# taleinat/fuzzysearch

Hardware: NVIDIA H100
Metric: haystack_GB_per_s_scanned (higher is better)
Workload: dtype u8

## Files before the change

fuzzysearch_b200/csrc/api.cu:

```cuda
#include <algorithm>
#include <atomic>
#include <cstdarg>
#include <cstdio>
#include <cmath>
#include <cstring>
#include <dlfcn.h>
#include <sched.h>
#include <unistd.h>
#include <condition_variable>
#include <memory>
#include <mutex>
#include <thread>
#include <new>
#include <string>
#include <type_traits>
#include <vector>

#include "kernels.cuh"
#include "ham_kernels.cuh"
#include "lp_kernels.cuh"
#include "post_kernels.cuh"
#include "p2p_kernels.cuh"
#include "batch_kernels.cuh"
#include "ham_batch_kernels.cuh"
// ... 8 lines not shown

static thread_local std::string g_err;

static int fail(int code, const char *fmt, ...) {
    char buf[512];
    va_list ap;
    va_start(ap, fmt);
    vsnprintf(buf, sizeof buf, fmt, ap);
    va_end(ap);
    g_err = buf;
    return code;
}

#define CK(call)                                                                          \
    do {                                                                                  \
        cudaError_t e_ = (call);                                                          \
        if (e_ != cudaSuccess)                                                            \
            return fail(FZB_E_CUDA, "%s failed: %s", #call, cudaGetErrorString(e_));      \
    } while (0)

#define TRY(call)                                                                         \
    do {                                                                                  \
        const int rc_ = (call);                                                           \
        if (rc_) return rc_;                                                              \
    } while (0)

enum class Mem { Device, Pinned, Mapped };

template <class T, Mem kMem>
class Buf {
  public:
    Buf() = default;
    Buf(Buf &&o) noexcept : p_(o.p_), n_(o.n_) {
        o.p_ = nullptr;
        o.n_ = 0;
    }
    Buf &operator=(Buf o) noexcept {
        std::swap(p_, o.p_);
        std::swap(n_, o.n_);
        return *this;
    }
    ~Buf() {
        if (p_) (void)(kMem == Mem::Device ? cudaFree(p_) : cudaFreeHost(p_));
    }
    T *get() const { return p_; }
    uint64_t size() const { return n_; }
    explicit operator bool() const { return p_ != nullptr; }
    T &operator[](uint64_t i) const {
        static_assert(kMem != Mem::Device, "device memory is not addressable from the host");
        return p_[i];
    }
    int alloc(uint64_t n, uint64_t bytes = 0) {
        Buf b;
        if (!bytes) bytes = n * sizeof(T);
        const unsigned flags = kMem == Mem::Mapped ? cudaHostAllocMapped | cudaHostAllocPortable : cudaHostAllocDefault;
        const cudaError_t e = kMem == Mem::Device ? cudaMalloc(&b.p_, bytes) : cudaHostAlloc(&b.p_, bytes, flags);
        if (e != cudaSuccess)
            return fail(FZB_E_CUDA, "%s(%llu bytes) failed: %s", kMem == Mem::Device ? "cudaMalloc" : "cudaHostAlloc",
                        (unsigned long long)bytes, cudaGetErrorString(e));
        b.n_ = n;
        *this = std::move(b);
        return FZB_OK;
    }

  private:
    T *p_ = nullptr;
    uint64_t n_ = 0;
};
template <class T> using DevBuf = Buf<T, Mem::Device>;
template <class T> using PinnedBuf = Buf<T, Mem::Pinned>;
template <class T> using MappedBuf = Buf<T, Mem::Mapped>;

struct BatchBufs {
    DevBuf<uint32_t> d_mbits;
    DevBuf<uint2> d_gtab;
    DevBuf<uint32_t> d_postings, d_pinfo;
    DevBuf<BatchPat> d_bpats;
    DevBuf<unsigned long long> d_mset;
    DevBuf<WorkItem> d_mwork;
};
struct LpBatchBufs {
    DevBuf<ulonglong2> d_lmlut;
    DevBuf<unsigned long long> d_lmlist;
    DevBuf<unsigned long long> d_lmkept;
    DevBuf<uint32_t> d_lmhist;
};
struct GenericBatchBufs {
    DevBuf<uint32_t> d_glim;
};
struct PeerBufs {
    DevBuf<uint8_t> d_p2p;
    DevBuf<MergeScratch> d_ms;
    DevBuf<unsigned long long> d_mscore;
    DevBuf<uint32_t> d_mpos;
    MappedBuf<int64_t> h_grows;
    MappedBuf<uint32_t> h_ghdr;
};
struct RecBufs {
    DevBuf<uint64_t> d_off;
    DevBuf<uint32_t> d_first;
    uint64_t longest = 0;
};
struct BestBufs {
    DevBuf<uint64_t> d_words;
    DevBuf<uint32_t> d_ids;
};
struct BestState {
    uint64_t *best, *top2;
    const uint32_t *ordinal;
};
struct NearBufs {
    DevBuf<uint64_t> d_head;
    DevBuf<uint64_t> d_words;
};
struct NearBatchBufs {
    DevBuf<uint32_t> d_lanes;
    DevBuf<uint8_t> d_pats;
    DevBuf<uint64_t> d_words;
    DevBuf<uint64_t> d_aux;
};
struct GatherBufs {
    uint32_t cap = 0;
    DevBuf<int64_t> d_send, d_recv;
    PinnedBuf<int64_t> h_send, h_recv;
};

template <class G, class F>
static int ensure_group(std::unique_ptr<G> &slot, F init) {
    if (slot) return FZB_OK;
    std::unique_ptr<G> g(new (std::nothrow) G());
    if (!g) return fail(FZB_E_CUDA, "out of host memory");
    TRY(init(*g));
    slot = std::move(g);
    return FZB_OK;
}

extern "C" int fzb_version(void) { return FZB_VERSION; }

extern "C" int fzb_device_count(void) {
    int n = 0;
    if (cudaGetDeviceCount(&n) != cudaSuccess) {
        cudaGetLastError();
        return 0;
    }
    return n;
}

extern "C" const char *fzb_last_error(void) { return g_err.c_str(); }

struct NcclId {
    char b[FZB_NCCL_ID_BYTES];
};
struct NcclApi {
    int (*GetUniqueId)(NcclId *id) = nullptr;
    int (*CommInitRank)(void **comm, int nranks, NcclId id, int rank) = nullptr;
    int (*AllGather)(const void *send, void *recv, size_t count, int dtype, void *comm, cudaStream_t s) = nullptr;
    int (*CommDestroy)(void *comm) = nullptr;
    const char *(*GetErrorString)(int) = nullptr;
    bool ok = false;
};
static NcclApi g_nccl;
static std::string g_nccl_path;

extern "C" void fzb_nccl_set_library(const char *path) { g_nccl_path = path ? path : ""; }

static int nccl_load() {
    static std::once_flag once;
// ... 1822 lines not shown
        if (rc > 0)
            for (uint32_t id : ids) drop(id);
        return rc < 0 ? rc : FZB_OK;
    }

    int finish_pass(const std::vector<RawRec> &raw, uint32_t n, const std::vector<uint32_t> &ids, fzb_stats pass,
                    int raw_order, bool unconsolidated) {
        if (!best) return split_batch(raw, ids, pass, raw_order, unconsolidated, out, &sum);
        if (n) {
            std::vector<uint32_t> ordinals(ids.size());
            for (size_t j = 0; j < ids.size(); j++) ordinals[j] = best->ordinal[ids[j]];
            CK(cudaMemcpyAsync(h->bestb->d_ids.get(), ordinals.data(), ordinals.size() * sizeof(uint32_t),
                               cudaMemcpyHostToDevice, h->stream));
            TRY(best_accumulate(h, *best, n, h->bestb->d_ids.get(), 0));
            pass.n_launches++;
        }
        for (uint32_t id : ids) done[id] = 1;
        add_stats(&sum, pass);
        return FZB_OK;
    }

    int finish(fzb_stats *total) {
        const uint32_t f = (flags & ~FZB_F_PER_RECORD) | (best ? FZB_F_NO_FINAL : 0u);
        for (uint32_t i = 0; i < count; i++) {
            if (settled(i)) continue;
            fzb_result *res = nullptr;
            auto planned = [&](Plan &pl) { pl = plans[i]; return FZB_OK; };
            TRY(settle(run_search(h, patterns + offsets[i], f, &res, planned), {}));
            if (!best) {
                add_stats(&sum, res->stats);
                out[i] = res;
                continue;
            }
            const int rc = best_accumulate(h, *best, res->raw_n, nullptr, best->ordinal[i]);
            if (res->raw_n) res->stats.n_launches++;
            add_stats(&sum, res->stats);
            fzb_result_destroy(res);
            TRY(rc);
        }
        sum.route = 7;
        if (total) *total = sum;
        return FZB_OK;
    }
};

template <class F>
static int run_batch_pass(const BatchCall &c, F enqueue, std::vector<RawRec> &raw, uint32_t cnts[CNT_COUNT],
                          fzb_stats &pass) {
    fzb_haystack *h = c.h;
    detach_pending(h);
    for (int attempt = 0; attempt < 8; attempt++) {
        h->counters_clean = false;
        CK(cudaMemsetAsync(h->d_counters.get(), 0, CNT_COUNT * sizeof(uint32_t), h->stream));
        CK(cudaEventRecord(h->ev[0], h->stream));
        int rc = enqueue();
        if (rc) return rc;
        CK(cudaEventRecord(h->ev[2], h->stream));
        rc = read_counters(h, cnts);
        if (rc) return rc;
        if (cnts[CNT_OVERFLOW]) return 1;
        const uint32_t n = cnts[CNT_OUT];
        if (n > kMaxRawRecs) return 1;
        if (n > h->d_out.size()) {
            TRY(ensure_out_cap(h, n));
            continue;
        }
        if (!c.best) raw.resize(n);
        if (!raw.empty()) {
            CK(cudaMemcpyAsync(raw.data(), h->d_out.get(), (size_t)n * sizeof(RawRec), cudaMemcpyDeviceToHost, h->stream));
            CK(cudaStreamSynchronize(h->stream));
        }
        float ms = 0.f;
        cudaEventElapsedTime(&ms, h->ev[0], h->ev[2]);
        pass.gpu_ms = ms;
        pass.bytes_scanned = h->buf_len;
        return FZB_OK;
    }
    return fail(FZB_E_CUDA, "output buffer kept overflowing");
}

struct ChunkSums {
    float scan_ms = 0.f;
    uint64_t listed = 0;
    uint32_t chunks = 0;
};

template <class S, class V>
static int run_chunks(fzb_haystack *h, uint64_t chunk, int list, int full, uint32_t cnts[CNT_COUNT], ChunkSums &s,
                      S scan, V verify) {
    s = ChunkSums{};
    for (uint64_t lo = h->own_lo; lo < h->own_hi; lo += chunk) {
        CK(cudaMemsetAsync(h->d_counters.get() + list, 0, 2 * sizeof(uint32_t), h->stream));
        CK(cudaEventRecord(h->ev[1], h->stream));
        scan(lo, std::min<uint64_t>(h->own_hi, lo + chunk));
        CK(cudaEventRecord(h->ev[2], h->stream));
        TRY(verify());
        CK(cudaGetLastError());
        s.chunks++;
        TRY(read_counters(h, cnts));
        float ms = 0.f;
        cudaEventElapsedTime(&ms, h->ev[1], h->ev[2]);
        s.scan_ms += ms;
        s.listed += cnts[list];
        if (cnts[CNT_OVERFLOW] || cnts[full]) return 1;
    }
    return FZB_OK;
}

static void fill_pat(BatchPat &bp, const BatchCall &c, uint32_t id) {
    memset(&bp, 0, sizeof bp);
    memcpy(bp.P, c.patterns + c.offsets[id], c.len(id));
    bp.m = (int)c.len(id);
    bp.k = (int)c.plans[id].k;
}

template <class F>
static int upload_pass_tables(fzb_haystack *h, const std::unordered_map<uint32_t, std::vector<uint32_t>> &grams,
                              const std::vector<uint32_t> &bits, const std::vector<uint32_t> &pinfo,
                              const std::vector<BatchPat> &pats, F mark) {
    std::vector<uint32_t> postings;
    std::vector<uint2> gtab(kGtabSlots, make_uint2(0, 0));
    for (auto &g : grams) {
        const uint32_t w = g.first;
        mark(w);
        for (size_t first = 0; first < g.second.size(); first += 255) {
            const uint32_t c = (uint32_t)std::min<size_t>(255, g.second.size() - first);
            uint32_t slot = (w * kGramMul) & (kGtabSlots - 1);
            while (gtab[slot].y != 0u) slot = (slot + 1) & (kGtabSlots - 1);
            gtab[slot] = make_uint2(w, (uint32_t)postings.size() | (c << 24));
            postings.insert(postings.end(), g.second.begin() + first, g.second.begin() + first + c);
        }
    }
    TRY(ensure_batch_buffers(h));
    BatchBufs &b = *h->batch;
    CK(cudaMemcpyAsync(b.d_mbits.get(), bits.data(), bits.size() * 4, cudaMemcpyHostToDevice, h->stream));
    CK(cudaMemcpyAsync(b.d_gtab.get(), gtab.data(), gtab.size() * sizeof(uint2), cudaMemcpyHostToDevice, h->stream));
    CK(cudaMemcpyAsync(b.d_postings.get(), postings.data(), postings.size() * 4, cudaMemcpyHostToDevice, h->stream));
    CK(cudaMemcpyAsync(b.d_pinfo.get(), pinfo.data(), pinfo.size() * 4, cudaMemcpyHostToDevice, h->stream));
    CK(cudaMemcpyAsync(b.d_bpats.get(), pats.data(), pats.size() * sizeof(BatchPat), cudaMemcpyHostToDevice, h->stream));
    return FZB_OK;
}

static MultiParams pass_params(const fzb_haystack *h) {
    MultiParams mp{};
    mp.H = h->d;
    mp.buf_lo = (int64_t)h->buf_lo;
    mp.buf_len = (int64_t)h->buf_len;
    mp.N = (int64_t)h->global_len;
    mp.own_lo = (int64_t)h->own_lo;
    mp.own_hi = (int64_t)h->own_hi;
    mp.bits = h->batch->d_mbits.get();
    mp.gtab = h->batch->d_gtab.get();
    mp.gtab_mask = kGtabSlots - 1;
    mp.postings = h->batch->d_postings.get();
    mp.pinfo = h->batch->d_pinfo.get();
    mp.counters = h->d_counters.get();
    return mp;
}

constexpr int kGenericBatchCap = 256;

static int prepare_generic_pass(const BatchCall &c, const std::vector<uint32_t> &ids, int grid) {
    fzb_haystack *h = c.h;
    TRY(ensure_group(h->gbatch, [](GenericBatchBufs &g) -> int { return g.d_glim.alloc(kMaxBatchPats); }));
    std::vector<uint32_t> lim;
    for (uint32_t id : ids) lim.push_back(c.plans[id].subs | c.plans[id].ins << 8 | c.plans[id].dels << 16);
    CK(cudaMemcpyAsync(h->gbatch->d_glim.get(), lim.data(), lim.size() * 4, cudaMemcpyHostToDevice, h->stream));
    return ensure_scratch(h, (uint64_t)grid * kLpThreads * 2 * kGenericBatchCap);
}

static int ensure_mhits(fzb_haystack *h) {
    if (h->d_mhits) return FZB_OK;
    DevBuf<unsigned long long> hits;
    TRY(hits.alloc(1u << 23));
    CK(cudaFuncSetAttribute(k_filter_mdense, cudaFuncAttributeMaxDynamicSharedMemorySize, (int)kMdenseSmem));
    h->d_mhits = std::move(hits);
    return FZB_OK;
}

static void two_bit_code(const uint8_t *patterns, const uint32_t *offsets, const std::vector<uint32_t> &ids,
                         uint8_t code[256]) {
    uint64_t freq[256] = {0};
    for (uint32_t id : ids)
        for (uint32_t b = offsets[id]; b < offsets[id + 1]; b++) freq[patterns[b]]++;
    int order[256];
    for (int c = 0; c < 256; c++) order[c] = c;
// ... 64 lines not shown
    const int64_t nvec = (int64_t)(round_up(h->buf_len, 16) / 16);
    const int64_t ntiles = (nvec + kMultiTileVecs - 1) / kMultiTileVecs;
    std::vector<RawRec> raw;
    uint32_t cnts[CNT_COUNT];
    fzb_stats pass{};
    const RecSet rs = rec_set(h);
    rc = run_batch_pass(c, [&]() -> int {
        MdenseParams dp{mp, b.d_bpats.get(), h->d_mhits.get(), hits_cap};
        if (ntiles > 0) {
            const int grid = (int)std::min<int64_t>(ntiles, h->sm_count);
            if (dense)
                k_filter_mdense<<<grid, kMultiThreads, kMdenseSmem, h->stream>>>(dp, nvec, ntiles);
            else
                k_filter_multi<<<grid, kMultiThreads, kMultiSmem, h->stream>>>(mp, nvec, ntiles);
        }
        CK(cudaEventRecord(h->ev[1], h->stream));
        with_recs(h, [&](auto rec) {
            constexpr bool R = decltype(rec)::value;
            if (generic && dense)
                k_verify_mhits_generic<R><<<ggrid, kLpThreads, 0, h->stream>>>(
                    dp, h->gbatch->d_glim.get(), h->d_scratch.get(), kGenericBatchCap, h->d_out.get(), h->d_out.size(),
                    h->d_counters.get(), rs);
            else if (generic)
                k_verify_multi_generic<R><<<ggrid, kLpThreads, 0, h->stream>>>(
                    mp, b.d_bpats.get(), h->gbatch->d_glim.get(), h->d_scratch.get(), kGenericBatchCap, h->d_out.get(),
                    h->d_out.size(), h->d_counters.get(), rs);
            else if (dense)
                k_verify_mhits<R><<<h->sm_count * 8, kMhThreads, 0, h->stream>>>(dp, h->d_out.get(), h->d_out.size(),
                                                                                    h->d_counters.get(), rs);
            else
                k_verify_multi<R><<<h->sm_count * 8, kVmThreads, 0, h->stream>>>(
                    mp, b.d_bpats.get(), h->d_out.get(), h->d_out.size(), h->d_counters.get(), rs);
        });
        CK(cudaGetLastError());
        return FZB_OK;
    }, raw, cnts, pass);
    if (rc > 0 && !dense) {
        CK(cudaMemsetAsync(b.d_mset.get(), 0, b.d_mset.size() * sizeof(unsigned long long), h->stream));
        CK(cudaStreamSynchronize(h->stream));
    }
    if (rc) return rc;
    float filter_ms = 0.f;
    cudaEventElapsedTime(&filter_ms, h->ev[0], h->ev[1]);
    pass.route = generic ? 9 : dense ? 2 : 1;
    pass.filter_ms = filter_ms;
    pass.n_candidates = cnts[CNT_CAND];
    pass.n_launches = 2;
    return c.finish_pass(raw, cnts[CNT_OUT], ids, pass, generic ? 2 : 0, false);
}

static int batch_pass_lp(BatchCall &c, const std::vector<uint32_t> &ids) {
    fzb_haystack *h = c.h;
    const uint32_t cnt = (uint32_t)ids.size();
    const bool generic = c.plans[ids[0]].generic();
    std::vector<BatchPat> pats(cnt);
    std::vector<ulonglong2> lut(256, make_ulonglong2(0ull, 0ull));
    std::vector<uint32_t> pm32((size_t)cnt * 256, 0u);
    LpMultiParams lp{};
    int wmax = 0;
    uint32_t kmax = 0;
    for (uint32_t i = 0; i < cnt; i++) {
        const uint32_t id = ids[i], m = c.len(id), k = c.plans[id].k;
        BatchPat &bp = pats[i];
        fill_pat(bp, c, id);
        for (uint32_t j = 0; j < m; j++) {
            lut[bp.P[j]].x |= 1ull << i;
            pm32[(size_t)i * 256 + bp.P[j]] |= 1u << j;
        }
        if (generic)
            for (int c = 0; c < 256; c++) lut[c].y |= 1ull << i;
        else
            for (uint32_t j = 0; j <= std::min(k, m - 1); j++) lut[bp.P[j]].y |= 1ull << i;
        const uint32_t bias = 32 - (m - k);
        for (int b = 0; b < 6; b++)
            if ((bias >> b) & 1u) lp.bias[b] |= 1ull << i;
        wmax = std::max(wmax, (int)(m + k));
        kmax = std::max(kmax, k);
    }
    TRY(ensure_batch_buffers(h));
    TRY(ensure_group(h->lpb, [&](LpBatchBufs &l) -> int {
        TRY(l.d_lmlut.alloc(256, 256 * sizeof(ulonglong2) + 64 * 256 * sizeof(uint32_t)));
        const uint64_t list_cap = std::min<uint64_t>(1u << 26, std::max<uint64_t>(1u << 22, h->owned_buf.size() / 16));
        TRY(l.d_lmlist.alloc(list_cap));
        TRY(l.d_lmkept.alloc(list_cap));
        TRY(l.d_lmhist.alloc(256));
        CK(cudaFuncSetAttribute(k_lp_scan_multi, cudaFuncAttributeMaxDynamicSharedMemorySize, (int)kLmSmem));
        return FZB_OK;
    }));
    LpBatchBufs &lb = *h->lpb;
    CK(cudaMemcpyAsync(lb.d_lmlut.get(), lut.data(), 256 * sizeof(ulonglong2), cudaMemcpyHostToDevice, h->stream));
    uint32_t *d_pm32 = reinterpret_cast<uint32_t *>(lb.d_lmlut.get() + 256);
    CK(cudaMemcpyAsync(d_pm32, pm32.data(), pm32.size() * sizeof(uint32_t), cudaMemcpyHostToDevice, h->stream));
    CK(cudaMemcpyAsync(h->batch->d_bpats.get(), pats.data(), pats.size() * sizeof(BatchPat), cudaMemcpyHostToDevice, h->stream));
    lp.H = h->d;
    lp.buf_lo = (int64_t)h->buf_lo;
    lp.buf_len = (int64_t)h->buf_len;
    lp.N = (int64_t)h->global_len;
    lp.lut = lb.d_lmlut.get();
    lp.wmax = wmax;
    lp.pats = h->batch->d_bpats.get();
    lp.pm32 = d_pm32;
    lp.list = lb.d_lmlist.get();
    lp.list_cap = c.tiny ? std::min<uint32_t>(lb.d_lmlist.size(), kTinyLpListCap) : (uint32_t)lb.d_lmlist.size();
    lp.counters = h->d_counters.get();
    int per_sm = 2;
    CK(cudaOccupancyMaxActiveBlocksPerMultiprocessor(&per_sm, k_lp_scan_multi, kLmThreads, kLmSmem));
    per_sm = std::max(per_sm, 1);
    const int vgrid = h->sm_count * 4, sim_cap = 256;
    if (generic)
        TRY(prepare_generic_pass(c, ids, vgrid));
    else
        TRY(ensure_scratch(h, (uint64_t)vgrid * kLpThreads * 2 * sim_cap));
    const uint64_t chunk = c.tiny ? kTinyLpChunk : 256ull << 20;
    std::vector<RawRec> raw;
    uint32_t cnts[CNT_COUNT];
    fzb_stats pass{};
    const RecSet rs = rec_set(h);
    ChunkSums cs;
    int rc = run_batch_pass(c, [&]() -> int {
        return run_chunks(h, chunk, CNT_LMLIST, CNT_LMWORK, cnts, cs, [&](uint64_t lo, uint64_t hi) {
            lp.own_lo = (int64_t)lo;
            lp.own_hi = (int64_t)hi;
            k_lp_scan_multi<<<h->sm_count * per_sm, kLmThreads, kLmSmem, h->stream>>>(lp);
        }, [&]() -> int {
            CK(cudaMemsetAsync(h->d_counters.get() + CNT_LMNEXT, 0, sizeof(uint32_t), h->stream));
            CK(cudaMemsetAsync(lb.d_lmhist.get(), 0, 256 * sizeof(uint32_t), h->stream));
            k_lm_refine<<<h->sm_count * 8, kLmSortThreads, 0, h->stream>>>(lp, lb.d_lmkept.get(), lb.d_lmhist.get());
            k_lm_scatter<<<h->sm_count * 8, kLmSortThreads, 0, h->stream>>>(lb.d_lmkept.get(), lb.d_lmhist.get(),
                                                                              lb.d_lmhist.get() + 128, lb.d_lmlist.get());
            with_recs(h, [&](auto rec) {
                constexpr bool R = decltype(rec)::value;
                if (generic)
                    k_lp_verify_multi_generic<R><<<vgrid, kLpThreads, 0, h->stream>>>(
                        lp, h->gbatch->d_glim.get(), lb.d_lmlist.get(), lb.d_lmhist.get(), h->d_scratch.get(),
                        kGenericBatchCap, h->d_out.get(), h->d_out.size(), h->d_counters.get(), rs);
                else if (kmax <= 4)
                    k_lp_verify_multi<4, R><<<vgrid, kLpThreads, 0, h->stream>>>(
                        lp, lb.d_lmlist.get(), lb.d_lmhist.get(), h->d_scratch.get(), sim_cap, h->d_out.get(),
                        h->d_out.size(), h->d_counters.get(), rs);
                else
                    k_lp_verify_multi<8, R><<<vgrid, kLpThreads, 0, h->stream>>>(
                        lp, lb.d_lmlist.get(), lb.d_lmhist.get(), h->d_scratch.get(), sim_cap, h->d_out.get(),
                        h->d_out.size(), h->d_counters.get(), rs);
            });
            return FZB_OK;
        });
    }, raw, cnts, pass);
    if (rc) return rc;
    pass.route = generic ? 10 : 3;
    pass.filter_ms = cs.scan_ms;
    pass.n_candidates = cs.listed;
    pass.n_launches = 4 * cs.chunks;
    return c.finish_pass(raw, cnts[CNT_OUT], ids, pass, 1, false);
}

constexpr double kDnaLevPostNs = 0.53;
constexpr double kDnaLevHitNs = 0.31;
constexpr double kDnaLevAloneMs = 0.13;
constexpr double kDnaLevAloneReadNs = 4.3e-4;
constexpr double kDnaLevAloneHitNs = 0.29;
constexpr double kDnaLevPassHits = 4.0;
constexpr uint32_t kDnaLevMinL = 5;

static uint32_t dna_lev_postings(const Plan &p) {
    return (p.m / p.L()) << (2 * (kHbKeySyms - std::min<uint32_t>(p.L(), kHbKeySyms)));
}

static double dna_lev_hits(const fzb_haystack *h, const Plan &p, double positions, bool *rides) {
    const uint32_t L = p.L(), n = p.m / L;
    const double c = h->coll_prob;
    const double post = n * std::pow(std::max(c, 0.25), (double)std::min<uint32_t>(L, kHbKeySyms));
    const double hits = n * std::pow(c, (double)L);
    const double pass_ns = positions * (kDnaLevPostNs * post + kDnaLevHitNs * hits);
    const double alone_ns = kDnaLevAloneMs * 1e6 + positions * (kDnaLevAloneReadNs + kDnaLevAloneHitNs * hits);
    *rides = pass_ns < alone_ns;
    return hits;
}

static int batch_pass_dna(BatchCall &c, const std::vector<uint32_t> &ids, double hits_per_pos) {
    fzb_haystack *h = c.h;
    const uint32_t cnt = (uint32_t)ids.size();
    std::vector<BatchPat> pats(cnt);
    std::vector<uint32_t> pinfo(cnt);
    Mdense2Params p{};
    two_bit_code(c.patterns, c.offsets, ids, p.code);
    std::unordered_map<uint32_t, std::vector<uint32_t>> keys;
    keys.reserve(cnt * 64);
    for (uint32_t i = 0; i < cnt; i++) {
        const uint32_t id = ids[i], m = c.len(id), k = c.plans[id].k;
        BatchPat &bp = pats[i];
        fill_pat(bp, c, id);
        bp.L = (int)c.plans[id].L();
        bp.n_ngrams = (int)m / bp.L;
        pinfo[i] = m | (k << 8) | ((uint32_t)bp.L << 16);
        for (int j = 0; j < bp.n_ngrams; j++) two_bit_key(keys, p.code, bp.P + j * bp.L, bp.L, (i << 8) | (uint32_t)j);
    }
    std::vector<uint32_t> bits(kHbKeyWords, 0);
    int rc = upload_pass_tables(h, keys, bits, pinfo, pats, [&](uint32_t w) { bits[w >> 5] |= 1u << (w & 31u); });
    if (rc) return rc;
    TRY(ensure_mhits(h));
    const uint32_t hits_cap = c.tiny ? std::min<uint32_t>(h->d_mhits.size(), kTinyBatchCap) : (uint32_t)h->d_mhits.size();
    p.dp = MdenseParams{pass_params(h), h->batch->d_bpats.get(), h->d_mhits.get(), hits_cap};
    const uint64_t tile = (uint64_t)kMultiTileVecs * 16;
    const uint64_t chunk = c.tiny ? kTinyLpChunk
                                  : std::max(tile, (uint64_t)(hits_cap / 2 / std::max(hits_per_pos, 1e-9)) / tile * tile);
    const int64_t nvec = (int64_t)(round_up(h->buf_len, 16) / 16);
    std::vector<RawRec> raw;
    uint32_t cnts[CNT_COUNT];
    fzb_stats pass{};
    const RecSet rs = rec_set(h);
    ChunkSums cs;
    rc = run_batch_pass(c, [&]() -> int {
        return run_chunks(h, chunk, CNT_MHITS, CNT_OVERFLOW, cnts, cs, [&](uint64_t lo, uint64_t hi) {
            p.scan_lo = (int64_t)lo;
            p.scan_hi = (int64_t)hi;
            const int64_t v0 = (p.scan_lo - (int64_t)h->buf_lo) / 16;
            const int64_t v1 = (p.scan_hi - (int64_t)h->buf_lo + 15) / 16;
            const int64_t ntiles = (v1 - v0 + kMultiTileVecs - 1) / kMultiTileVecs;
            p.dp.mp.counters = h->d_counters.get();
            k_filter_mdense2<<<(int)std::min<int64_t>(ntiles, h->sm_count), kMultiThreads, kMdense2Smem, h->stream>>>(
                p, nvec, v0, ntiles);
        }, [&]() -> int {
            with_recs(h, [&](auto rec) {
                constexpr bool R = decltype(rec)::value;
                k_verify_mhits<R><<<h->sm_count * 8, kMhThreads, 0, h->stream>>>(p.dp, h->d_out.get(), h->d_out.size(),
                                                                                    h->d_counters.get(), rs);
            });
            return FZB_OK;
        });
    }, raw, cnts, pass);
    if (rc) return rc;
// ... 1075 lines not shown
```

fuzzysearch_b200/csrc/batch_kernels.cuh:

```cuda
#pragma once
#include "lp_kernels.cuh"

namespace fzb {

constexpr int kMultiThreads = 1024;
constexpr int kMultiTblBits = 20;
constexpr int kMultiTblWords = 1 << (kMultiTblBits - 5);
constexpr size_t kMultiSmem = (size_t)kMultiTblWords * 4;
constexpr int kMultiUnroll = 4;
constexpr int kMultiTileVecs = kMultiThreads * kMultiUnroll;
constexpr uint32_t kGramMul = 0x85EBCA77u;
constexpr int kMulti2Bits = 23;
constexpr int kMulti2Words = 1 << (kMulti2Bits - 5);
constexpr uint32_t kGramMul2 = 0xC2B2AE35u;
__host__ __device__ __forceinline__ uint32_t multi_hash2(uint32_t w) { return ((w ^ (w >> 15)) * kGramMul2) >> (32 - kMulti2Bits); }
constexpr int kBatchMaxM = 64;

struct BatchPat {
    uint8_t P[kBatchMaxM];
    int32_t m, k, L, n_ngrams;
};

struct WorkItem {
    uint32_t pid, granule, slot, pad;
// ... 312 lines not shown
                full |= mdense2_confirm(dp, sBuf, sN, (uint32_t)(codes >> (2 * b)) & 0xFFFFu, g0 + b);
            }
        }
        if (__syncthreads_or(full)) {
            flush_cta_buffer(sBuf, sN, min(*sN, (uint32_t)kMdBuf), &sBase, dp.hits, dp.hits_cap,
                             &dp.mp.counters[CNT_MHITS], kMultiThreads);
            __syncthreads();
        }
    }
    __syncthreads();
    const uint32_t n = min(*sN, (uint32_t)kMdBuf);
    if (n) flush_cta_buffer(sBuf, sN, n, &sBase, dp.hits, dp.hits_cap, &dp.mp.counters[CNT_MHITS], kMultiThreads);
}

constexpr int kMhThreads = 128;
constexpr int kMhSlotBytes = 160;

template <bool REC>
__global__ void __launch_bounds__(kMhThreads)
k_verify_mhits(const __grid_constant__ MdenseParams p, RawRec *out, uint32_t cap, uint32_t *counters, const RecSet rs) {
    __shared__ __align__(16) uint8_t slots[kMhThreads][kMhSlotBytes];
    __shared__ __align__(16) uint8_t pats[kMhThreads][kBatchMaxM];
    const uint32_t nhits = counters[CNT_MHITS];
    if (nhits > p.hits_cap) {
        if (blockIdx.x == 0 && threadIdx.x == 0) counters[CNT_OVERFLOW] = 1;
        return;
    }
    const int lane = threadIdx.x & 31;
    uint8_t *slot = slots[threadIdx.x];
    uint8_t *myP = pats[threadIdx.x];
    for (;;) {
        uint32_t base = 0;
        if (lane == 0) base = atomicAdd(&counters[CNT_MHITWORK], 32u);
        base = __shfl_sync(0xFFFFFFFFu, base, 0);
        if (base >= nhits) break;
        const uint32_t item = base + lane;
        bool valid = item < nhits;
        VerifyCtx c;
        c.H = p.mp.H;
        c.buf_lo = p.mp.buf_lo;
        c.buf_len = p.mp.buf_len;
        c.N = p.mp.N;
        c.own_lo = p.mp.own_lo;
        c.own_hi = p.mp.own_hi;
        c.m = c.k = 1;
        c.L = 1;
        c.n_ngrams = 1;
        int64_t idx = 0, alo = 0, lo = 0, hi = 0;
        int j = 0, tag = 0;
        if (valid) {
            const unsigned long long hv = p.hits[item];
            idx = p.mp.buf_lo + (int64_t)(hv & ((1ull << 40) - 1));
            j = (int)((hv >> 40) & 0xFFu);
            const uint32_t pid = (uint32_t)(hv >> 48);
            tag = (int)(pid << 8);
            const BatchPat *bp = p.pats + pid;
            c.m = bp->m;
            c.k = bp->k;
            c.L = bp->L;
            c.n_ngrams = bp->n_ngrams;
            for (int w = 0; w < kBatchMaxM / 4; w++)
                reinterpret_cast<uint32_t *>(myP)[w] = __ldg(reinterpret_cast<const uint32_t *>(bp->P) + w);
            if constexpr (REC) {
                valid = rec_bounds(rs, idx, lo, hi);
                if (valid) alo = stage_lane_window(c, idx - (int64_t)j * c.L, slot, lo, hi);
            } else {
                alo = stage_lane_window(c, idx - (int64_t)j * c.L, slot);
            }
        }
        verify_anchor_lev<3, REC>(c, myP, nullptr, slot - alo, idx, valid, nullptr, out, cap, counters, j, j + 1, tag,
                                  lo, hi);
    }
    if (blockIdx.x == 0 && threadIdx.x == 0) atomicAdd(&counters[CNT_CAND], nhits);
}

constexpr int kLmThreads = 256;
constexpr int kLmRun = 128;
constexpr int kLmTile = kLmThreads * kLmRun;
constexpr int kLmHalo = 64;
constexpr int kLmBuf = 6144;
constexpr int kLmFlush = 2048;
constexpr size_t kLmTileBytes = ((size_t)(kLmTile + kLmHalo) / 128 * 132 + 132 + 15) / 16 * 16;
constexpr size_t kLmSmem = kLmTileBytes + 256 * 16 + (size_t)kLmBuf * 8 + 16;
enum { CNT_LMLIST = 7, CNT_LMWORK = 8 };

struct LpMultiParams {
    const uint8_t *H;
    int64_t buf_lo, buf_len, N, own_lo, own_hi;
    const ulonglong2 *lut;
    unsigned long long bias[6];
    int wmax;
    const BatchPat *pats;
    const uint32_t *pm32;
    unsigned long long *list;
    uint32_t list_cap;
    uint32_t *counters;
};

__device__ __forceinline__ uint32_t lm_addr(uint32_t i) { return i + 4u * (i >> 7); }

__global__ void __launch_bounds__(kLmThreads)
k_lp_scan_multi(const __grid_constant__ LpMultiParams p) {
    extern __shared__ __align__(16) uint8_t lm_smem[];
    uint8_t *sH = lm_smem;
    ulonglong2 *sLut = reinterpret_cast<ulonglong2 *>(lm_smem + kLmTileBytes);
    unsigned long long *sBuf = reinterpret_cast<unsigned long long *>(sLut + 256);
    uint32_t *sN = reinterpret_cast<uint32_t *>(sBuf + kLmBuf);
    __shared__ uint32_t sBase;
    for (int i = threadIdx.x; i < 256; i += kLmThreads) sLut[i] = p.lut[i];
    if (threadIdx.x == 0) *sN = 0;
    __syncthreads();
    const int64_t hi = min(p.own_hi, p.N);
    const int64_t lim = min(p.N, p.buf_lo + p.buf_len);
    const int64_t base = p.own_lo & ~(int64_t)127;
    const int64_t ntiles = hi > base ? (hi - base + kLmTile - 1) / kLmTile : 0;
    const int wmax = p.wmax;
    for (int64_t t = blockIdx.x; t < ntiles; t += gridDim.x) {
        const int64_t tile_lo = base + t * kLmTile;
        __syncthreads();
        {
            const int nwords = (kLmTile + kLmHalo) / 4;
            const uint8_t *src = p.H + (tile_lo - p.buf_lo);
            const int64_t first = p.buf_lo - tile_lo;
            const int64_t avail = p.buf_lo + p.buf_len + 128 - tile_lo;
            for (int w = threadIdx.x; w < nwords; w += kLmThreads) {
                const int64_t b = (int64_t)w * 4;
                const uint32_t v = (b >= first && b + 4 <= avail) ? __ldg(reinterpret_cast<const uint32_t *>(src + b)) : 0u;
                *reinterpret_cast<uint32_t *>(sH + lm_addr((uint32_t)w * 4u)) = v;
            }
        }
        __syncthreads();
        const uint32_t r0 = threadIdx.x * kLmRun;
        const int64_t s0 = tile_lo + r0;
        unsigned long long C[6];
#pragma unroll
        for (int i = 0; i < 6; i++) C[i] = p.bias[i];
        for (int j = 0; j < wmax; j++) {
            unsigned long long carry = (s0 + j < lim) ? sLut[sH[lm_addr(r0 + j)]].x : 0ull;
#pragma unroll
            for (int i = 0; i < 6; i++) {
                const unsigned long long c = C[i];
                C[i] = c ^ carry;
                carry &= c;
            }
        }
        for (int r = 0; r < kLmRun; r++) {
            const int64_t s = s0 + r;
            ulonglong2 lf = make_ulonglong2(0ull, 0ull);
            if (s < lim) lf = sLut[sH[lm_addr(r0 + r)]];
            unsigned long long surv = C[5] & lf.y;
            if (surv && s >= p.own_lo && s < hi) {
                const uint32_t n = (uint32_t)__popcll(surv);
                uint32_t slot = atomicAdd(sN, n);
                while (surv) {
                    const int pid = __ffsll((long long)surv) - 1;
                    surv &= surv - 1;
                    const unsigned long long ent = (unsigned long long)(s - p.buf_lo) | ((unsigned long long)pid << 40);
                    if (slot < (uint32_t)kLmBuf) {
                        sBuf[slot] = ent;
                    } else {
                        const uint32_t g = atomicAdd(&p.counters[CNT_LMLIST], 1u);
                        if (g < p.list_cap) p.list[g] = ent;
                    }
                    slot++;
                }
            }
            const unsigned long long ae = (s + wmax < lim) ? sLut[sH[lm_addr(r0 + r + wmax)]].x : 0ull;
            unsigned long long up = ae & ~lf.x, dn = lf.x & ~ae;
#pragma unroll
            for (int i = 0; i < 6; i++) {
                const unsigned long long c = C[i];
                C[i] = c ^ up ^ dn;
                up &= c;
                dn &= ~c;
            }
        }
        __syncthreads();
        const uint32_t n = min(*sN, (uint32_t)kLmBuf);
        if (n >= (uint32_t)kLmFlush)
            flush_cta_buffer(sBuf, sN, n, &sBase, p.list, p.list_cap, &p.counters[CNT_LMLIST], kLmThreads);
    }
    __syncthreads();
    const uint32_t n = min(*sN, (uint32_t)kLmBuf);
    if (n) flush_cta_buffer(sBuf, sN, n, &sBase, p.list, p.list_cap, &p.counters[CNT_LMLIST], kLmThreads);
}

constexpr int kLmSortThreads = 256;

__global__ void __launch_bounds__(kLmSortThreads)
k_lm_refine(const __grid_constant__ LpMultiParams p, unsigned long long *kept, uint32_t *hist ) {
    __shared__ uint32_t sHist[64];
    __shared__ unsigned long long sKeep[kLmSortThreads];
    __shared__ unsigned long long sA[256];
    __shared__ uint32_t sN, sBase;
    const uint32_t n = p.counters[CNT_LMLIST];
    if (n > p.list_cap) return;
    for (int i = threadIdx.x; i < 256; i += kLmSortThreads) sA[i] = p.lut[i].x;
    const uint8_t *W = p.H - p.buf_lo;
    const int64_t lim = min(p.N, p.buf_lo + p.buf_len);
    if (threadIdx.x < 64) sHist[threadIdx.x] = 0;
    for (uint32_t base = blockIdx.x * kLmSortThreads; base < n; base += gridDim.x * kLmSortThreads) {
        if (threadIdx.x == 0) sN = 0;
        __syncthreads();
        const uint32_t i = base + threadIdx.x;
        if (i < n) {
            const unsigned long long ent = p.list[i];
            const int64_t st = p.buf_lo + (int64_t)(ent & ((1ull << 40) - 1));
            const uint32_t pid = (uint32_t)(ent >> 40);
            const BatchPat *bp = p.pats + pid;
            const int m = bp->m, k = bp->k, win = m + k, need = m - k;
            int cnt = 0;
            for (int j = 0; j < win && st + j < lim; j++) cnt += (int)((sA[W[st + j]] >> pid) & 1ull);
            if (cnt >= need) {
                sKeep[atomicAdd(&sN, 1u)] = ent;
                atomicAdd(&sHist[pid], 1u);
            }
        }
        __syncthreads();
        const uint32_t kn = sN;
        if (kn) {
            if (threadIdx.x == 0) sBase = atomicAdd(&hist[64], kn);
            __syncthreads();
            if (threadIdx.x < kn) kept[sBase + threadIdx.x] = sKeep[threadIdx.x];
        }
        __syncthreads();
    }
    __syncthreads();
    if (threadIdx.x < 64 && sHist[threadIdx.x]) atomicAdd(&hist[threadIdx.x], sHist[threadIdx.x]);
}

__global__ void __launch_bounds__(kLmSortThreads)
k_lm_scatter(const unsigned long long *kept, const uint32_t *hist, uint32_t *cursors, unsigned long long *sorted) {
    __shared__ uint32_t sOff[64], sCnt[64], sBase[64];
    const uint32_t n = hist[64];
    if (threadIdx.x == 0) {
        uint32_t acc = 0;
        for (int q = 0; q < 64; q++) {
            sOff[q] = acc;
            acc += hist[q];
        }
    }
    for (uint32_t base = blockIdx.x * kLmSortThreads; base < n; base += gridDim.x * kLmSortThreads) {
        if (threadIdx.x < 64) sCnt[threadIdx.x] = 0;
        __syncthreads();
        const uint32_t i = base + threadIdx.x;
        unsigned long long ent = 0;
        uint32_t pid = 0, rank = 0;
        if (i < n) {
            ent = kept[i];
            pid = (uint32_t)(ent >> 40);
            rank = atomicAdd(&sCnt[pid], 1u);
        }
        __syncthreads();
        if (threadIdx.x < 64 && sCnt[threadIdx.x]) sBase[threadIdx.x] = atomicAdd(&cursors[threadIdx.x], sCnt[threadIdx.x]);
        __syncthreads();
        if (i < n) sorted[sOff[pid] + sBase[pid] + rank] = ent;
        __syncthreads();
    }
}

struct LpLaneCtx {
    int32_t m, k;
    int64_t N;
};

enum { CNT_LMNEXT = 10 };

template <int K, bool REC>
__global__ void __launch_bounds__(kLpThreads)
k_lp_verify_multi(const __grid_constant__ LpMultiParams p, const unsigned long long *sorted, const uint32_t *hist,
                  uint32_t *scratch, int cap, RawRec *out, uint32_t ocap, uint32_t *counters, const RecSet rs) {
    __shared__ __align__(4) uint8_t sPat[kLpThreads][kBatchMaxM / 2];
    if (counters[CNT_LMLIST] > p.list_cap) {
        if (blockIdx.x == 0 && threadIdx.x == 0) counters[CNT_LMWORK] = 1;
        return;
    }
    const uint32_t n = hist[64];
    const int64_t tid = (int64_t)blockIdx.x * blockDim.x + threadIdx.x;
    const int lane = threadIdx.x & 31;
    uint32_t *A = scratch + tid * 2 * (int64_t)cap, *B = A + cap;
    const uint8_t *W = p.H - p.buf_lo;
    uint8_t *myP = sPat[threadIdx.x];
    bool have = false, drained = false;
    int64_t st = 0, i = 0;
    uint32_t pid = 0;
    LpLaneCtx c;
    c.m = 2;
    c.k = 1;
    c.N = p.N;
    const uint32_t *pm = p.pm32;
    uint32_t R[K + 1];
#pragma unroll
    for (int d = 0; d <= K; d++) R[d] = 0;
    for (;;) {
        const unsigned want = __ballot_sync(0xFFFFFFFFu, !have && !drained);
        bool accept = false;
        if (want) {
            const int leader = __ffs(want) - 1;
            uint32_t base = 0;
            if (lane == leader) base = atomicAdd(&counters[CNT_LMNEXT], (uint32_t)__popc(want));
            base = __shfl_sync(0xFFFFFFFFu, base, leader);
            if (!have && !drained) {
                const uint32_t idx = base + (uint32_t)__popc(want & ((1u << lane) - 1u));
                if (idx >= n) {
                    drained = true;
                } else {
                    const unsigned long long ent = sorted[idx];
                    st = p.buf_lo + (int64_t)(ent & ((1ull << 40) - 1));
                    pid = (uint32_t)(ent >> 40);
                    const BatchPat *bp = p.pats + pid;
                    c.m = bp->m;
                    c.k = bp->k;
                    pm = p.pm32 + (size_t)pid * 256;
                    for (int w = 0; w < kBatchMaxM / 8; w++)
                        reinterpret_cast<uint32_t *>(myP)[w] = __ldg(reinterpret_cast<const uint32_t *>(bp->P) + w);
                    int j0 = -1;
                    const uint8_t ch = W[st];
                    for (int j = 0; j <= min(c.k, c.m - 1); j++)
                        if (myP[j] == ch) {
                            j0 = j;
                            break;
                        }
                    if constexpr (REC) {
                        int64_t lo;
                        if (!rec_bounds(rs, st, lo, c.N)) j0 = -1;
                    }
                    if (j0 >= 0) {
                        if (j0 + 1 == c.m) {
                            accept = true;
                        } else {
#pragma unroll
                            for (int d = 0; d <= K; d++) R[d] = (d == j0) ? (1u << (j0 + 1)) : 0u;
                            i = st + 1;
                            have = true;
                        }
                    }
                }
            }
        }
        if (__all_sync(0xFFFFFFFFu, drained && !have && !accept)) break;
        if (have) {
            if (i >= (REC ? c.N : p.N)) {
                accept = lp_nfa_end<K>(R, c.m, c.k);
                have = false;
            } else {
                bool alive = true;
                if (lp_nfa_step<K>(R, __ldg(pm + W[i]), i + 1 < (REC ? c.N : p.N), c.m, c.k, alive)) {
                    accept = true;
                    have = false;
// ... 66 lines not shown
```

Baseline: 2615.

## Fuse candidate window refinement into the LP scan kernel using the shared-memory tile

The separate k_lm_refine kernel is removed. Its windowed count test now runs inside k_lp_scan_multi against the tile already staged in shared memory, and the per-pattern histogram is built there too. A small k_lm_offsets kernel does a warp-shuffle prefix sum to produce scatter cursors, so k_lm_scatter no longer computes offsets serially. This cuts a kernel launch and a second pass over the candidate list and haystack in global memory. In exchange the scan kernel gains extra shared memory, barriers and retest work per tile.

```diff
diff --git a/fuzzysearch_b200/csrc/api.cu b/fuzzysearch_b200/csrc/api.cu
--- a/fuzzysearch_b200/csrc/api.cu
+++ b/fuzzysearch_b200/csrc/api.cu
@@ -114,7 +114,7 @@
 struct LpBatchBufs {
     DevBuf<ulonglong2> d_lmlut;
     DevBuf<unsigned long long> d_lmlist;
-    DevBuf<unsigned long long> d_lmkept;
+    DevBuf<unsigned long long> d_lmsorted;
     DevBuf<uint32_t> d_lmhist;
 };
 struct GenericBatchBufs {
@@ -2103,6 +2103,7 @@
 struct ChunkSums {
     float scan_ms = 0.f;
     uint64_t listed = 0;
+    uint64_t kept = 0;
     uint32_t chunks = 0;
 };
 
@@ -2111,7 +2112,7 @@
                       S scan, V verify) {
     s = ChunkSums{};
     for (uint64_t lo = h->own_lo; lo < h->own_hi; lo += chunk) {
-        CK(cudaMemsetAsync(h->d_counters.get() + list, 0, 2 * sizeof(uint32_t), h->stream));
+        CK(cudaMemsetAsync(h->d_counters.get() + list, 0, 3 * sizeof(uint32_t), h->stream));
         CK(cudaEventRecord(h->ev[1], h->stream));
         scan(lo, std::min<uint64_t>(h->own_hi, lo + chunk));
         CK(cudaEventRecord(h->ev[2], h->stream));
@@ -2123,6 +2124,7 @@
         cudaEventElapsedTime(&ms, h->ev[1], h->ev[2]);
         s.scan_ms += ms;
         s.listed += cnts[list];
+        s.kept += cnts[list + 2];
         if (cnts[CNT_OVERFLOW] || cnts[full]) return 1;
     }
     return FZB_OK;
@@ -2353,7 +2355,7 @@
         TRY(l.d_lmlut.alloc(256, 256 * sizeof(ulonglong2) + 64 * 256 * sizeof(uint32_t)));
         const uint64_t list_cap = std::min<uint64_t>(1u << 26, std::max<uint64_t>(1u << 22, h->owned_buf.size() / 16));
         TRY(l.d_lmlist.alloc(list_cap));
-        TRY(l.d_lmkept.alloc(list_cap));
+        TRY(l.d_lmsorted.alloc(list_cap));
         TRY(l.d_lmhist.alloc(256));
         CK(cudaFuncSetAttribute(k_lp_scan_multi, cudaFuncAttributeMaxDynamicSharedMemorySize, (int)kLmSmem));
         return FZB_OK;
@@ -2388,36 +2390,37 @@
     fzb_stats pass{};
     const RecSet rs = rec_set(h);
     ChunkSums cs;
+    uint32_t *hist = lb.d_lmhist.get(), *cursors = hist + 128;
     int rc = run_batch_pass(c, [&]() -> int {
+        CK(cudaMemsetAsync(hist, 0, 64 * sizeof(uint32_t), h->stream));
         return run_chunks(h, chunk, CNT_LMLIST, CNT_LMWORK, cnts, cs, [&](uint64_t lo, uint64_t hi) {
             lp.own_lo = (int64_t)lo;
             lp.own_hi = (int64_t)hi;
-            k_lp_scan_multi<<<h->sm_count * per_sm, kLmThreads, kLmSmem, h->stream>>>(lp);
+            k_lp_scan_multi<<<h->sm_count * per_sm, kLmThreads, kLmSmem, h->stream>>>(lp, hist);
         }, [&]() -> int {
-            CK(cudaMemsetAsync(h->d_counters.get() + CNT_LMNEXT, 0, sizeof(uint32_t), h->stream));
-            CK(cudaMemsetAsync(lb.d_lmhist.get(), 0, 256 * sizeof(uint32_t), h->stream));
-            k_lm_refine<<<h->sm_count * 8, kLmSortThreads, 0, h->stream>>>(lp, lb.d_lmkept.get(), lb.d_lmhist.get());
-            k_lm_scatter<<<h->sm_count * 8, kLmSortThreads, 0, h->stream>>>(lb.d_lmkept.get(), lb.d_lmhist.get(),
-                                                                              lb.d_lmhist.get() + 128, lb.d_lmlist.get());
+            k_lm_offsets<<<1, 64, 0, h->stream>>>(hist, cursors, h->d_counters.get(), lp.list_cap);
+            k_lm_scatter<<<h->sm_count * 8, kLmSortThreads, 0, h->stream>>>(lb.d_lmlist.get(), hist, cursors,
+                                                                              lb.d_lmsorted.get());
             with_recs(h, [&](auto rec) {
                 constexpr bool R = decltype(rec)::value;
                 if (generic)
                     k_lp_verify_multi_generic<R><<<vgrid, kLpThreads, 0, h->stream>>>(
-                        lp, h->gbatch->d_glim.get(), lb.d_lmlist.get(), lb.d_lmhist.get(), h->d_scratch.get(),
+                        lp, h->gbatch->d_glim.get(), lb.d_lmsorted.get(), hist, h->d_scratch.get(),
                         kGenericBatchCap, h->d_out.get(), h->d_out.size(), h->d_counters.get(), rs);
                 else if (kmax <= 4)
                     k_lp_verify_multi<4, R><<<vgrid, kLpThreads, 0, h->stream>>>(
-                        lp, lb.d_lmlist.get(), lb.d_lmhist.get(), h->d_scratch.get(), sim_cap, h->d_out.get(),
+                        lp, lb.d_lmsorted.get(), hist, h->d_scratch.get(), sim_cap, h->d_out.get(),
                         h->d_out.size(), h->d_counters.get(), rs);
                 else
                     k_lp_verify_multi<8, R><<<vgrid, kLpThreads, 0, h->stream>>>(
-                        lp, lb.d_lmlist.get(), lb.d_lmhist.get(), h->d_scratch.get(), sim_cap, h->d_out.get(),
+                        lp, lb.d_lmsorted.get(), hist, h->d_scratch.get(), sim_cap, h->d_out.get(),
                         h->d_out.size(), h->d_counters.get(), rs);
             });
             return FZB_OK;
         });
     }, raw, cnts, pass);
     if (rc) return rc;
+    h->h_counters[CNT_LMKEPT] = (uint32_t)std::min<uint64_t>(cs.kept, UINT32_MAX);
     pass.route = generic ? 10 : 3;
     pass.filter_ms = cs.scan_ms;
     pass.n_candidates = cs.listed;
diff --git a/fuzzysearch_b200/csrc/batch_kernels.cuh b/fuzzysearch_b200/csrc/batch_kernels.cuh
--- a/fuzzysearch_b200/csrc/batch_kernels.cuh
+++ b/fuzzysearch_b200/csrc/batch_kernels.cuh
@@ -418,7 +418,8 @@
 constexpr int kLmFlush = 2048;
 constexpr size_t kLmTileBytes = ((size_t)(kLmTile + kLmHalo) / 128 * 132 + 132 + 15) / 16 * 16;
 constexpr size_t kLmSmem = kLmTileBytes + 256 * 16 + (size_t)kLmBuf * 8 + 16;
-enum { CNT_LMLIST = 7, CNT_LMWORK = 8 };
+enum { CNT_LMLIST = 7, CNT_LMWORK = 8, CNT_LMKEPT = 9, CNT_LMNEXT = 10  };
+constexpr int kLmRetest = 4;
 
 struct LpMultiParams {
     const uint8_t *H;
@@ -435,17 +436,37 @@
 
 __device__ __forceinline__ uint32_t lm_addr(uint32_t i) { return i + 4u * (i >> 7); }
 
+__device__ __forceinline__ int lm_in(const uint8_t *sH, const ulonglong2 *sLut, uint32_t r, int pid) {
+    return (int)(sLut[sH[lm_addr(r)]].x >> pid) & 1;
+}
+
+__device__ __forceinline__ bool lm_own_window(const uint8_t *sH, const ulonglong2 *sLut, uint32_t r, int64_t s,
+                                              int pid, int w, int need, int64_t lim) {
+    int cnt = 0;
+    for (int j = 0; j < w && s + j < lim; j++) cnt += lm_in(sH, sLut, r + (uint32_t)j, pid);
+    return cnt >= need;
+}
+
 __global__ void __launch_bounds__(kLmThreads)
-k_lp_scan_multi(const __grid_constant__ LpMultiParams p) {
+k_lp_scan_multi(const __grid_constant__ LpMultiParams p, uint32_t *hist) {
     extern __shared__ __align__(16) uint8_t lm_smem[];
     uint8_t *sH = lm_smem;
     ulonglong2 *sLut = reinterpret_cast<ulonglong2 *>(lm_smem + kLmTileBytes);
     unsigned long long *sBuf = reinterpret_cast<unsigned long long *>(sLut + 256);
     uint32_t *sN = reinterpret_cast<uint32_t *>(sBuf + kLmBuf);
-    __shared__ uint32_t sBase;
+    __shared__ uint32_t sBase, sKept;
+    __shared__ uint32_t sHist[64];
+    __shared__ uint8_t sWin[64], sNeed[64];
     for (int i = threadIdx.x; i < 256; i += kLmThreads) sLut[i] = p.lut[i];
+    if (threadIdx.x < 64) {
+        sHist[threadIdx.x] = 0;
+        const BatchPat &bp = p.pats[threadIdx.x];
+        sWin[threadIdx.x] = (uint8_t)(bp.m + bp.k);
+        sNeed[threadIdx.x] = (uint8_t)(bp.m - bp.k);
+    }
     if (threadIdx.x == 0) *sN = 0;
     __syncthreads();
+    const int lane = threadIdx.x & 31;
     const int64_t hi = min(p.own_hi, p.N);
     const int64_t lim = min(p.N, p.buf_lo + p.buf_len);
     const int64_t base = p.own_lo & ~(int64_t)127;
@@ -454,6 +475,8 @@
     for (int64_t t = blockIdx.x; t < ntiles; t += gridDim.x) {
         const int64_t tile_lo = base + t * kLmTile;
         __syncthreads();
+        const uint32_t t0 = *sN;
+        if (threadIdx.x == 0) sKept = t0;
         {
             const int nwords = (kLmTile + kLmHalo) / 4;
             const uint8_t *src = p.H + (tile_lo - p.buf_lo);
@@ -494,9 +517,10 @@
                     const unsigned long long ent = (unsigned long long)(s - p.buf_lo) | ((unsigned long long)pid << 40);
                     if (slot < (uint32_t)kLmBuf) {
                         sBuf[slot] = ent;
-                    } else {
-                        const uint32_t g = atomicAdd(&p.counters[CNT_LMLIST], 1u);
+                    } else if (lm_own_window(sH, sLut, r0 + r, s, pid, sWin[pid], sNeed[pid], lim)) {
+                        const uint32_t g = atomicAdd(&p.counters[CNT_LMKEPT], 1u);
                         if (g < p.list_cap) p.list[g] = ent;
+                        atomicAdd(&sHist[pid], 1u);
                     }
                     slot++;
                 }
@@ -512,70 +536,92 @@
             }
         }
         __syncthreads();
-        const uint32_t n = min(*sN, (uint32_t)kLmBuf);
+        const uint32_t nraw = *sN, n1 = min(nraw, (uint32_t)kLmBuf);
+        for (uint32_t b = t0; b < n1; b += kLmThreads * kLmRetest) {
+            unsigned long long ent[kLmRetest];
+            uint32_t r[kLmRetest];
+            int pid[kLmRetest], cnt[kLmRetest], jn[kLmRetest], span = 0;
+#pragma unroll
+            for (int e = 0; e < kLmRetest; e++) {
+                const uint32_t i = b + (uint32_t)(e * kLmThreads) + threadIdx.x;
+                ent[e] = i < n1 ? sBuf[i] : 0ull;
+                const int64_t s = p.buf_lo + (int64_t)(ent[e] & ((1ull << 40) - 1));
+                pid[e] = (int)(ent[e] >> 40);
+                r[e] = (uint32_t)(s - tile_lo);
+                const int w = sWin[pid[e]];
+                cnt[e] = i >= n1 ? -1 : w == wmax ? 64 : -(int)sNeed[pid[e]];
+                jn[e] = (i < n1 && w < wmax) ? (int)min((int64_t)w, lim - s) : 0;
+                span = max(span, jn[e]);
+            }
+            for (int j = 0; j < span; j++) {
+#pragma unroll
+                for (int e = 0; e < kLmRetest; e++)
+                    if (j < jn[e]) cnt[e] += lm_in(sH, sLut, r[e] + (uint32_t)j, pid[e]);
+            }
+            unsigned km[kLmRetest];
+            uint32_t nk = 0;
+#pragma unroll
+            for (int e = 0; e < kLmRetest; e++) {
+                km[e] = __ballot_sync(0xFFFFFFFFu, cnt[e] >= 0);
+                nk += (uint32_t)__popc(km[e]);
+            }
+            __syncthreads();
+            uint32_t dst = 0;
+            if (lane == 0 && nk) dst = atomicAdd(&sKept, nk);
+            dst = __shfl_sync(0xFFFFFFFFu, dst, 0);
+#pragma unroll
+            for (int e = 0; e < kLmRetest; e++) {
+                if ((km[e] >> lane) & 1u) {
+                    sBuf[dst + (uint32_t)__popc(km[e] & ((1u << lane) - 1u))] = ent[e];
+                    atomicAdd(&sHist[pid[e]], 1u);
+                }
+                dst += (uint32_t)__popc(km[e]);
+            }
+        }
+        __syncthreads();
+        const uint32_t n = sKept;
+        if (threadIdx.x == 0) {
+            atomicAdd(&p.counters[CNT_LMLIST], nraw - t0);
+            *sN = n;
+        }
         if (n >= (uint32_t)kLmFlush)
-            flush_cta_buffer(sBuf, sN, n, &sBase, p.list, p.list_cap, &p.counters[CNT_LMLIST], kLmThreads);
-    }
-    __syncthreads();
-    const uint32_t n = min(*sN, (uint32_t)kLmBuf);
-    if (n) flush_cta_buffer(sBuf, sN, n, &sBase, p.list, p.list_cap, &p.counters[CNT_LMLIST], kLmThreads);
+            flush_cta_buffer(sBuf, sN, n, &sBase, p.list, p.list_cap, &p.counters[CNT_LMKEPT], kLmThreads);
+    }
+    __syncthreads();
+    const uint32_t n = *sN;
+    if (n) flush_cta_buffer(sBuf, sN, n, &sBase, p.list, p.list_cap, &p.counters[CNT_LMKEPT], kLmThreads);
+    __syncthreads();
+    if (threadIdx.x < 64 && sHist[threadIdx.x]) atomicAdd(&hist[threadIdx.x], sHist[threadIdx.x]);
 }
 
 constexpr int kLmSortThreads = 256;
 
+__global__ void __launch_bounds__(64)
+k_lm_offsets(uint32_t *hist, uint32_t *cursors, uint32_t *counters, uint32_t list_cap) {
+    const uint32_t q = threadIdx.x, lane = q & 31;
+    __shared__ uint32_t sWarp[2];
+    const uint32_t c = hist[q];
+    uint32_t incl = c;
+#pragma unroll
+    for (int d = 1; d < 32; d *= 2) {
+        const uint32_t v = __shfl_up_sync(0xFFFFFFFFu, incl, d);
+        if (lane >= (uint32_t)d) incl += v;
+    }
+    if (lane == 31) sWarp[q >> 5] = incl;
+    __syncthreads();
+    if (q >= 32) incl += sWarp[0];
+    cursors[q] = incl - c;
+    hist[q] = 0;
+    if (q == 63) {
+        hist[64] = counters[CNT_LMLIST] > list_cap ? 0u : incl;
+        counters[CNT_LMNEXT] = 0;
+    }
+}
+
 __global__ void __launch_bounds__(kLmSortThreads)
-k_lm_refine(const __grid_constant__ LpMultiParams p, unsigned long long *kept, uint32_t *hist ) {
-    __shared__ uint32_t sHist[64];
-    __shared__ unsigned long long sKeep[kLmSortThreads];
-    __shared__ unsigned long long sA[256];
-    __shared__ uint32_t sN, sBase;
-    const uint32_t n = p.counters[CNT_LMLIST];
-    if (n > p.list_cap) return;
-    for (int i = threadIdx.x; i < 256; i += kLmSortThreads) sA[i] = p.lut[i].x;
-    const uint8_t *W = p.H - p.buf_lo;
-    const int64_t lim = min(p.N, p.buf_lo + p.buf_len);
-    if (threadIdx.x < 64) sHist[threadIdx.x] = 0;
-    for (uint32_t base = blockIdx.x * kLmSortThreads; base < n; base += gridDim.x * kLmSortThreads) {
-        if (threadIdx.x == 0) sN = 0;
-        __syncthreads();
-        const uint32_t i = base + threadIdx.x;
-        if (i < n) {
-            const unsigned long long ent = p.list[i];
-            const int64_t st = p.buf_lo + (int64_t)(ent & ((1ull << 40) - 1));
-            const uint32_t pid = (uint32_t)(ent >> 40);
-            const BatchPat *bp = p.pats + pid;
-            const int m = bp->m, k = bp->k, win = m + k, need = m - k;
-            int cnt = 0;
-            for (int j = 0; j < win && st + j < lim; j++) cnt += (int)((sA[W[st + j]] >> pid) & 1ull);
-            if (cnt >= need) {
-                sKeep[atomicAdd(&sN, 1u)] = ent;
-                atomicAdd(&sHist[pid], 1u);
-            }
-        }
-        __syncthreads();
-        const uint32_t kn = sN;
-        if (kn) {
-            if (threadIdx.x == 0) sBase = atomicAdd(&hist[64], kn);
-            __syncthreads();
-            if (threadIdx.x < kn) kept[sBase + threadIdx.x] = sKeep[threadIdx.x];
-        }
-        __syncthreads();
-    }
-    __syncthreads();
-    if (threadIdx.x < 64 && sHist[threadIdx.x]) atomicAdd(&hist[threadIdx.x], sHist[threadIdx.x]);
-}
-
-__global__ void __launch_bounds__(kLmSortThreads)
-k_lm_scatter(const unsigned long long *kept, const uint32_t *hist, uint32_t *cursors, unsigned long long *sorted) {
-    __shared__ uint32_t sOff[64], sCnt[64], sBase[64];
+k_lm_scatter(const unsigned long long *list, const uint32_t *hist, uint32_t *cursors, unsigned long long *sorted) {
+    __shared__ uint32_t sCnt[64], sBase[64];
     const uint32_t n = hist[64];
-    if (threadIdx.x == 0) {
-        uint32_t acc = 0;
-        for (int q = 0; q < 64; q++) {
-            sOff[q] = acc;
-            acc += hist[q];
-        }
-    }
     for (uint32_t base = blockIdx.x * kLmSortThreads; base < n; base += gridDim.x * kLmSortThreads) {
         if (threadIdx.x < 64) sCnt[threadIdx.x] = 0;
         __syncthreads();
@@ -583,14 +629,14 @@
         unsigned long long ent = 0;
         uint32_t pid = 0, rank = 0;
         if (i < n) {
-            ent = kept[i];
+            ent = list[i];
             pid = (uint32_t)(ent >> 40);
             rank = atomicAdd(&sCnt[pid], 1u);
         }
         __syncthreads();
         if (threadIdx.x < 64 && sCnt[threadIdx.x]) sBase[threadIdx.x] = atomicAdd(&cursors[threadIdx.x], sCnt[threadIdx.x]);
         __syncthreads();
-        if (i < n) sorted[sOff[pid] + sBase[pid] + rank] = ent;
+        if (i < n) sorted[sBase[pid] + rank] = ent;
         __syncthreads();
     }
 }
@@ -600,7 +646,6 @@
     int64_t N;
 };
 
-enum { CNT_LMNEXT = 10 };
 
 template <int K, bool REC>
 __global__ void __launch_bounds__(kLpThreads)
```

After: 2606, median of 6. No clear change (-0.4%).
